# Sanoojan/REFace

Measured on AMD Instinct MI355X. Metric: 512x512 50-step DDIM images/sec, higher is better.
Workload: dtype bf16; 1 GPU; BASELINE configs[1]: 512x512, 50 DDIM steps, CFG scale 3.5, batch 8 per GPU, bf16 UNet + fp32 VAE decode (bf16x3 MFMA operands), seeded random-init REFace weights; id=c1:512x512:S50:B8:bf16, batch_per_gpu=8, global_batch=8, ddim_steps=50, latent=64, parallelism=dp1 (pairs sharded, no collective in the step loop)

## Files before the change

### reface_amd/csrc/common.h

```cpp
#pragma once
#include <hip/hip_runtime.h>
#include <stdint.h>
#include <stdio.h>
#include <stdlib.h>
#include <string.h>

#include "../../include/reface_hip.h"

typedef __attribute__((ext_vector_type(8))) __bf16 bf16x8_t;
typedef __attribute__((ext_vector_type(16))) float f32x16_t;
typedef __attribute__((ext_vector_type(4))) float f32x4_t;
typedef __attribute__((ext_vector_type(4))) uint32_t u32x4_t;
typedef __attribute__((ext_vector_type(2))) uint32_t u32x2_t;

typedef uint16_t bf16_t;
typedef _Float16 f16_t;
typedef __attribute__((ext_vector_type(8))) _Float16 f16x8_t;
typedef uint8_t fp8_t;

namespace rf {

void set_error(const char* fmt, ...);


// ... 117 lines not shown
template <> struct elem<f16_t> {
    static constexpr int VEC = 8;
    __device__ static __forceinline__ float load(const f16_t* p) { return (float)*p; }
    __device__ static __forceinline__ void store(f16_t* p, float v) { *p = (f16_t)v; }
};

template <typename T> __device__ __forceinline__ void unpack16(const u32x4_t& v, float* f);
template <> __device__ __forceinline__ void unpack16<float>(const u32x4_t& v, float* f) {
#pragma unroll
    for (int i = 0; i < 4; ++i) f[i] = as_f32( v[i]);
}
template <> __device__ __forceinline__ void unpack16<bf16_t>(const u32x4_t& v, float* f) {
#pragma unroll
    for (int i = 0; i < 4; ++i) {
        f[2 * i] = as_f32( v[i] << 16);
        f[2 * i + 1] = as_f32( v[i] & 0xffff0000u);
    }
}
template <> __device__ __forceinline__ void unpack16<f16_t>(const u32x4_t& v, float* f) {
#pragma unroll
    for (int i = 0; i < 4; ++i) {
        const uint32_t w = v[i];
        f[2 * i] = lo16<f16_t>(w);
        f[2 * i + 1] = hi16<f16_t>(w);
    }
}
template <typename T> __device__ __forceinline__ u32x4_t pack16(const float* f);
template <> __device__ __forceinline__ u32x4_t pack16<float>(const float* f) {
    u32x4_t v;
#pragma unroll
    for (int i = 0; i < 4; ++i) v[i] = as_u32( f[i]);
    return v;
}
template <> __device__ __forceinline__ u32x4_t pack16<bf16_t>(const float* f) {
    u32x4_t v;
#pragma unroll
    for (int i = 0; i < 4; ++i) v[i] = pack_bf2(f[2 * i], f[2 * i + 1]);
    return v;
}

template <> __device__ __forceinline__ u32x4_t pack16<f16_t>(const float* f) {
    u32x4_t v;
#pragma unroll
    for (int i = 0; i < 4; ++i) v[i] = pack_h2(f[2 * i], f[2 * i + 1]);
    return v;
}

template <typename T> __device__ __forceinline__ void mma16(f32x16_t& acc, const u32x4_t& a, const u32x4_t& b);
template <> __device__ __forceinline__ void mma16<bf16_t>(f32x16_t& acc, const u32x4_t& a, const u32x4_t& b) {
    acc = __builtin_amdgcn_mfma_f32_32x32x16_bf16(__builtin_bit_cast(bf16x8_t, a), __builtin_bit_cast(bf16x8_t, b), acc, 0, 0, 0);
}
template <> __device__ __forceinline__ void mma16<f16_t>(f32x16_t& acc, const u32x4_t& a, const u32x4_t& b) {
    acc = __builtin_amdgcn_mfma_f32_32x32x16_f16(__builtin_bit_cast(f16x8_t, a), __builtin_bit_cast(f16x8_t, b), acc, 0, 0, 0);
}

__device__ __forceinline__ float silu_exact(float x) {
    const float e = __builtin_amdgcn_exp2f(x * -1.4426950408889634f);
    return x * __builtin_amdgcn_rcpf(1.0f + e);
}
__device__ __forceinline__ float erf_rational(float x) {
    x = fminf(fmaxf(x, -4.0f), 4.0f);
    const float x2 = x * x;
    float a = -2.72614225801306e-10f;
    a = fmaf(a, x2, 2.77068142495902e-08f);
    a = fmaf(a, x2, -2.10102402082508e-06f);
    a = fmaf(a, x2, -5.69250639462346e-05f);
    a = fmaf(a, x2, -7.34990630326855e-04f);
    a = fmaf(a, x2, -2.95459980854025e-03f);
    a = fmaf(a, x2, -1.60960333262415e-02f);
    float b = -1.45660718464996e-05f;
    b = fmaf(b, x2, -2.13374055278905e-04f);
    b = fmaf(b, x2, -1.68282697438203e-03f);
    b = fmaf(b, x2, -7.37332916720468e-03f);
    b = fmaf(b, x2, -1.42647390514189e-02f);
    return x * a * __builtin_amdgcn_rcpf(b);
}
__device__ __forceinline__ float gelu_erf(float x) { return 0.5f * x * (1.0f + erf_rational(x * 0.70710678118654752440f)); }
__device__ __forceinline__ float gelu_sigmoid5(float x) {
    const float xc = __builtin_fminf(__builtin_fmaxf(x, -7.0f), 7.0f);
    const float x2 = xc * xc;
    const float u = xc * __builtin_fmaf(__builtin_fmaf(-0.0010142630f, x2, 0.10677572f), x2, 2.3011212f);
    return x * __builtin_amdgcn_rcpf(1.0f + __builtin_amdgcn_exp2f(-u));
}
template <typename T> __device__ __forceinline__ float gelu_for(float x) {
    if constexpr (sizeof(T) == 2) return gelu_sigmoid5(x);
    else return gelu_erf(x);
}
__device__ __forceinline__ float quick_gelu(float x) { return x / (1.0f + expf(-1.702f * x)); }

__device__ __forceinline__ void halfwave_reduce_scatter32(float (&gx)[32], int lrow) {
#pragma unroll
    for (int st = 0; st < 5; ++st) {
        const int m = 16 >> st, n = 16 >> st;
        const unsigned up = (lrow & m) ? 0xffffffffu : 0u;
#pragma unroll
        for (int k = 0; k < n; ++k) {
            const unsigned a = __float_as_uint(gx[k]), b = __float_as_uint(gx[k + n]);
            const float send = __uint_as_float((a & up) | (b & ~up));
            const float keep = __uint_as_float((b & up) | (a & ~up));
            gx[k] = keep + __shfl_xor(send, m, 64);
        }
    }
}

__device__ __forceinline__ float wave_sum(float v) {
    v += as_f32((uint32_t)__builtin_amdgcn_mov_dpp((int)as_u32(v), 0xB1, 0xF, 0xF, true));
// ... 36 lines not shown
```

### reface_amd/csrc/gemm.hip

```cpp
#include <cstdlib>
#include <type_traits>

#include "common.h"


namespace rf {
typedef float f32x2_t __attribute__((ext_vector_type(2)));

struct GemmParams {
    int M, N, K;
    const void* src0;
    const void* src1;
    int C0, Ctot, ld0, ld1;
    int Hin, Win, Hout, Wout, KH, KW, stride, pad_t, pad_l, ups;
    const void* W;
    int ldw;
    const float* bias;
    const float* rowvec;
    int rows_per_sample, ldv;
    const void* residual;
    int ldr, act;
    const float* act_vec;
    void* out;
    int ldo;
    float alpha;
    long long sA, sW, sO, sR;
    int tiles_m, tiles_n;
    unsigned a_bytes, w_bytes;
    int glds;
    int korder;
    int vec_ok;
    int splitk;
    float* ws;
    int pm, pn;
    int gn_rows;
    double* gn_part[2];
    int gn_cpg[2], gn_coff[2], gn_slot[2], gn_nch[2];
    int* plan;
    int epi2_ok;
    const float* wscale;
    void* oscale;
    int os_ld;
    const void* ascale;
    int as_ld;
    unsigned as_bytes;
    float* ln_out;
    int ln_out_parts;
    const float* ln_in;
    int ln_in_parts, ln_in_cols;
    float ln_eps;
    const float* ln_u;
    int x3;
    int lo_off;
    long long w_ps;
    const void* srcx;
    int ldx, xt0;
    unsigned x_bytes;
};

typedef __attribute__((ext_vector_type(2))) __bf16 bf16x2v_t;
__device__ __forceinline__ u32x4_t fp8x8_to_bf16x8(const u32x2_t& r, float scale) {
    u32x4_t o;
    o[0] = __builtin_bit_cast(uint32_t, __builtin_amdgcn_cvt_scalef32_pk_bf16_fp8(r[0], scale, false));
    o[1] = __builtin_bit_cast(uint32_t, __builtin_amdgcn_cvt_scalef32_pk_bf16_fp8(r[0], scale, true));
    o[2] = __builtin_bit_cast(uint32_t, __builtin_amdgcn_cvt_scalef32_pk_bf16_fp8(r[1], scale, false));
    o[3] = __builtin_bit_cast(uint32_t, __builtin_amdgcn_cvt_scalef32_pk_bf16_fp8(r[1], scale, true));
    return o;
}

template <typename T> struct MmaFrag;
template <> struct MmaFrag<bf16_t> {
    __device__ static __forceinline__ void mma(f32x16_t& acc, const u32x4_t& a, const u32x4_t& b) {
        acc = __builtin_amdgcn_mfma_f32_32x32x16_bf16(__builtin_bit_cast(bf16x8_t, a), __builtin_bit_cast(bf16x8_t, b), acc, 0, 0, 0);
    }
};
template <> struct MmaFrag<f16_t> {
    __device__ static __forceinline__ void mma(f32x16_t& acc, const u32x4_t& a, const u32x4_t& b) { mma16<f16_t>(acc, a, b); }
};
template <> struct MmaFrag<fp8_t> {
    __device__ static __forceinline__ void mma(f32x16_t&, const u32x4_t&, const u32x4_t&) {}
};
typedef int v8i_t __attribute__((ext_vector_type(8)));
__device__ __forceinline__ void mma_mx8(f32x16_t& acc, const u32x4_t& a0, const u32x4_t& a1, int sa, const u32x4_t& b0, const u32x4_t& b1, int sb) {
    const v8i_t a = {(int)a0[0], (int)a0[1], (int)a0[2], (int)a0[3], (int)a1[0], (int)a1[1], (int)a1[2], (int)a1[3]};
    const v8i_t b = {(int)b0[0], (int)b0[1], (int)b0[2], (int)b0[3], (int)b1[0], (int)b1[1], (int)b1[2], (int)b1[3]};
    asm volatile("s_nop 1\n\tv_mfma_scale_f32_32x32x64_f8f6f4 %0, %1, %2, %0, %3, %4 op_sel_hi:[0,0,0]" : "+v"(acc) : "v"(a), "v"(b), "v"(sa), "v"(sb));
}
template <> struct MmaFrag<float> {
    __device__ static __forceinline__ void mma(f32x16_t& acc, const u32x4_t& a, const u32x4_t& b) {
#pragma unroll
        for (int q = 0; q < 4; ++q)
            acc = __builtin_amdgcn_mfma_f32_32x32x2f32(as_f32( a[q]), as_f32( b[q]), acc, 0, 0, 0);
    }
};

__device__ __forceinline__ void lds_barrier() {
    asm volatile("s_waitcnt lgkmcnt(0)" ::: "memory");
    __builtin_amdgcn_s_barrier();
    asm volatile("" ::: "memory");
}

__device__ __forceinline__ int lds_off(int row, int slot) { return row * 128 + ((slot ^ ((row >> 1) & 7)) << 4); }

template <bool W8> __device__ __forceinline__ int w_stage(int t, int buf) { return W8 ? ((t >> 1) & 1) : buf; }
template <bool W8> __device__ __forceinline__ int w_soff(int t) { return (W8 ? (t >> 1) : t) * 128; }

template <typename TO> __device__ __forceinline__ void store_out(TO* p, float v);
template <> __device__ __forceinline__ void store_out<float>(float* p, float v) { *p = v; }
template <> __device__ __forceinline__ void store_out<bf16_t>(bf16_t* p, float v) { *p = f2bf(v); }
template <> __device__ __forceinline__ void store_out<f16_t>(f16_t* p, float v) { *p = (f16_t)v; }
template <typename TO> __device__ __forceinline__ float load_out(const TO* p);
template <> __device__ __forceinline__ float load_out<float>(const float* p) { return *p; }
template <> __device__ __forceinline__ float load_out<bf16_t>(const bf16_t* p) { return bf2f(*p); }
template <> __device__ __forceinline__ float load_out<f16_t>(const f16_t* p) { return (float)*p; }
template <typename X> struct is16 { static constexpr bool value = std::is_same<X, bf16_t>::value || std::is_same<X, f16_t>::value; };

template <typename T, typename TO, int WM, int WN, int TM, int TN, bool CONV, bool GLDS, int NST, int EPI = 0, bool W8 = false, int LNF = 0, bool HX = false>
__global__ __launch_bounds__(WM* WN * 64) void conv_gemm_kernel(const GemmParams p) {
    static_assert(LNF == 0 || (EPI == 1 && !CONV && !W8 && sizeof(T) == 2 && sizeof(TO) == 2), "LayerNorm folding: bf16 linear layers on the direct epilogue");
    static_assert(!HX || (CONV && GLDS && NST == 2 && sizeof(T) == 2 && !W8), "row-extended A tiles: bf16 3x3 convolutions on the two-stage direct-to-LDS loop");
    static_assert(EPI == 0 || GLDS, "the direct epilogue is built on the direct-to-LDS main loop");
    static_assert(!W8 || (GLDS && std::is_same<T, bf16_t>::value), "fp8 weights: bf16 activations on the direct-to-LDS main loop");
    constexpr bool A8 = std::is_same<T, fp8_t>::value;
    static_assert(!A8 || (GLDS && !W8 && NST == 2), "fp8 activations: direct-to-LDS main loop, two stages");
    constexpr int NT = WM * WN * 64;
    constexpr int BM = 32 * TM * WM;
    constexpr int BN = 32 * TN * WN;
    constexpr int VEC = elem<T>::VEC;
    constexpr int BK = 8 * VEC;
    constexpr int RPP = NT / 8;
    constexpr int AXR = HX ? ((BM * 5 / 4 + RPP - 1) / RPP) * RPP : BM;
    constexpr int AV = AXR / RPP;
    constexpr int BV = BN / RPP;
    static_assert(BM % RPP == 0 && BN % RPP == 0, "tile/threads mismatch");

    extern __shared__ __attribute__((aligned(16))) char smem[];
    char* const ldsA = smem;
    char* const ldsB = smem + NST * AXR * 128;
    char* const ldsS = smem + NST * (AXR + BN) * 128;

    const int tid = threadIdx.x;
    const int lane = tid & 63;
    const int wave = tid >> 6;
    const int wm = wave / WN, wn = wave % WN;

    int bid = blockIdx.x;
    {
        const int nwg = gridDim.x;
        const int q = nwg >> 3, r = nwg & 7, xcd = bid & 7, idx = bid >> 3;
        bid = (xcd < r ? xcd * (q + 1) : r * (q + 1) + (xcd - r) * q) + idx;
    }
    int tile_m, tile_n;
    {
        const int srow = p.pm * p.tiles_n;
        const int sr = bid / srow, rem = bid - sr * srow;
        const int h = min(p.pm, p.tiles_m - sr * p.pm);
        const int pw = h * p.pn;
        const int pc = rem / pw, r2 = rem - pc * pw;
        const int c = r2 / h;
        tile_m = sr * p.pm + (r2 - c * h);
        tile_n = pc * p.pn + c;
    }
    const int m0 = tile_m * BM, n0 = tile_n * BN;

    const long long zb = blockIdx.y;
    const T* src0 = (const T*)p.src0 + zb * p.sA;
    const T* src1 = (const T*)p.src1;
    const T* Wp = W8 ? (const T*)((const char*)p.W + zb * p.sW) : (const T*)p.W + zb * p.sW;
    if (!W8 && p.w_ps) Wp += (long long)(m0 / p.rows_per_sample) * p.w_ps;
    const int hw_in = p.Hin * p.Win;
    const int uph = (CONV && p.ups == 2) ? (m0 / hw_in) & 3 : 0;
// ... 368 lines not shown
                constexpr int cur = kk, nx = kk ^ 1, nkk = kk ^ 1;
                const char* const nA = kk == 0 ? curA : othA;
                const char* const nB = kk == 0 ? curB : othB;
                const char* const nS = kk == 0 ? curS : othS;
#pragma unroll
                for (int j = 0; j < JS8; ++j) mma_col(cur, j);
                if (kk == 1) {
                    asm volatile("s_waitcnt vmcnt(0) lgkmcnt(0)" ::: "memory");
                    __builtin_amdgcn_s_barrier();
                }
                ld_a(nx, nA, nS, nkk);
#pragma unroll
                for (int j = 0; j < JS8; ++j) ld_b(j, nB, nkk);
                __builtin_amdgcn_sched_barrier(0);
#pragma unroll
                for (int j = JS8; j < TN; ++j) {
                    mma_col(cur, j);
                    ld_b(j, nB, nkk);
                    if (kk == 1) {
                        constexpr int COLS = TN - JS8, PPC = (NP + COLS - 1) / COLS;
                        if (more) issue_pieces(stage, (j - JS8) * PPC, (j - JS8 + 1) * PPC < NP ? (j - JS8 + 1) * PPC : NP);
                    }
                    __builtin_amdgcn_sched_barrier(0);
                }
                __builtin_amdgcn_sched_barrier(0);
            };
            if (nk > 0) {
                issue_pieces(0, 0, AV);
                if (nk > 1) {
                    next_tile();
                    issue_pieces(1, 0, NP);
                    if (nk > 2) next_tile();
                    asm volatile("s_waitcnt vmcnt(%0)" ::"n"(NP + 1) : "memory");
                } else {
                    asm volatile("s_waitcnt vmcnt(0)" ::: "memory");
                }
                __builtin_amdgcn_s_barrier();
                ld_a(0, curA, curS, 0);
#pragma unroll
                for (int j = 0; j < TN; ++j) ld_b(j, curB, 0);
            }
            for (int kt = 0; kt < nk; ++kt) {
                const int stage = kt & 1;
                const bool more = kt + 2 < nk;
                phase8(integral_constant<int, 0>{}, stage, more);
                phase8(integral_constant<int, 1>{}, stage, more);
                if (kt + 3 < nk) next_tile();
                const char* t = curA; curA = othA; othA = t;
                t = curB; curB = othB; othB = t;
                t = curS; curS = othS; othS = t;
            }
            asm volatile("s_nop 15\n\ts_nop 15" ::: "memory");
            __syncthreads();
        } else {
        constexpr bool ROT = TM * TN > 8;
        constexpr int JS = ROT ? 2 : 0;
        u32x4_t fa[2][TM], fb[W8 ? 1 : 2][W8 ? 1 : TN];
        u32x2_t fbr[W8 ? 2 : 1][W8 ? TN : 1];
        float ws[W8 ? TN : 1];
        const int frag_sw = (lrow >> 1) & 7;
        const int brow = EPI == 1 ? (16 * ((lrow >> 2) & 1) + 4 * (lrow >> 3) + (lrow & 3)) : lrow;
        const int frag_swb = (brow >> 1) & 7;
        int fk[4], fkb[4];
#pragma unroll
        for (int kk = 0; kk < 4; ++kk) {
            fk[kk] = ((kk * 2 + lhalf) ^ frag_sw) << 4;
            fkb[kk] = W8 ? (((kk ^ frag_swb) << 4) + lhalf * 8) : (((kk * 2 + lhalf) ^ frag_swb) << 4);
        }
        if constexpr (W8) {
#pragma unroll
            for (int j = 0; j < TN; ++j) {
                const int n = n0 + (wn * TN + j) * 32 + brow;
                ws[j] = n < p.N ? p.wscale[n] : 1.0f;
            }
        }
        const char* curA = ldsA + (wm * TM) * 4096 + lrow * 128;
        int erow[TM];
        const char* hcb[TM];
        const char* hnb[TM];
        int hcs[TM], hns[TM], m_dx = 0, m_st = 0, m_len = 3, m_t = kb0_tiles;
        const int ks_[4] = {(0 + lhalf) << 4, (2 + lhalf) << 4, (4 + lhalf) << 4, (6 + lhalf) << 4};
        auto hx_set = [&](const char** hb, int* hs, int st, int dx) {
#pragma unroll
            for (int i = 0; i < TM; ++i) {
                const int e = erow[i] + dx;
                hb[i] = ldsA + st * (AXR * 128) + e * 128;
                hs[i] = ((e >> 1) & 7) << 4;
            }
        };
        if constexpr (HX) {
#pragma unroll
            for (int i = 0; i < TM; ++i) {
                const int pm = (wm * TM + i) * 32 + lrow, ir = pm / p.Wout;
                erow[i] = ir * (p.Wout + 2) + (pm - ir * p.Wout);
            }
            if (XT && kb0_tiles >= xt0) {
                m_len = 1;
                hx_set(hcb, hcs, 0, 1);
                hx_set(hnb, hns, 1, 1);
            } else {
                hx_set(hcb, hcs, 0, 0);
                hx_set(hnb, hns, 0, 1);
            }
        }
        const char* const wbase = ldsB + (wn * TN) * 4096 + brow * 128;
        const char* curB = wbase + w_stage<W8>(kb0_tiles, 0) * BN * 128;
// ... 927 lines not shown
            const double conc = 32.0, cap = 3.0 * 1024 * 1024;
            auto cost_of = [&](int h, int w) {
                const double nsr = (double)run / ((double)h * p.tiles_n) < 1.0 ? 1.0 : (double)run / ((double)h * p.tiles_n);
                const double npc = (double)p.tiles_n / w;
                const double a_t = (h * a_panel + w * w_panel <= cap) ? h * a_panel : npc * h * a_panel;
                return nsr * (a_t + p.tiles_n * w_panel);
            };
            double best = mfast ? cost_m : cost_n;
            const double strip_model = mfast ? cost_of(p.tiles_m, 1) : cost_of(1, p.tiles_n);
            if (strip_model > best) best = strip_model;
            for (int h = 2; h < p.tiles_m && h <= 32; h *= 2) {
                int w = (int)((conc + h - 1) / h);
                if (w < 1) w = 1;
                if (w >= p.tiles_n) continue;
                const double c = cost_of(h, w);
                if (c < 0.6 * best) { pm = h; pn = w; best = c / 0.6; }
            }
        }
        p.pm = pm;
        p.pn = pn;
    }
    constexpr bool FRAG_OK = (WM * WN == 8) || (TM * TN == 5) || (TM * TN >= 16) || std::is_same<T, fp8_t>::value;
    const bool frag = FRAG_OK && p.splitk > 1 && p.glds && p.epi2_ok && d->act == RF_ACT_NONE && !p.oscale && d->batch == 1 &&
                      (long long)p.splitk * p.tiles_m * p.tiles_n * BM * BN * 4 <= d->workspace_bytes;
    const int skr = sk_rows_for(p.M, p.N);
    const int st_rows = p.splitk > 1 ? (frag ? 32 : skr) : BM, st_cols = p.splitk > 1 ? (frag ? 32 * TN : SK_COLS) : BN;
    if (W8 || A8) RF_CHECK(p.glds, "rf_conv_gemm: fp8 operands need the direct-to-LDS main loop (one source, K and channel count multiples of the K tile)");
    if (p.oscale) {
        constexpr bool DOK = (WM * WN == 8) || (TM * TN == 5) || (TM * TN >= 16) || A8;
        RF_CHECK(DOK && TN % 2 == 0 && p.glds && p.epi2_ok && p.splitk == 1,
                 "rf_conv_gemm: fp8 output needs the direct epilogue (even TN, aligned rows, no split-K) -- this launch got a %d x %d tile", BM, BN);
    }
    constexpr bool DIRECT_OK = (WM * WN == 8) || (TM * TN == 5) || (TM * TN >= 16) || std::is_same<T, fp8_t>::value;
    const bool ep_common = p.glds && p.epi2_ok && p.splitk == 1 && (!p.rowvec || p.rows_per_sample % BM == 0) &&
                           (d->act == RF_ACT_NONE || d->act == RF_ACT_ADD_RELU || (d->act == RF_ACT_GEGLU && TN % 2 == 0));
    const bool direct = DIRECT_OK && ep_common && (p.gn_rows == 0 || d->act == RF_ACT_NONE);
    RF_CHECK(!hx || (HX_OK && conv && p.glds && p.KH == 3 && p.KW == 3 && p.stride == 1 && !p.ups && p.pad_t == 1 && p.pad_l == 1 && p.Hin == p.Hout &&
                     p.Win == p.Wout && p.Wout >= 16 && BM % p.Wout == 0 && (BM / p.Wout) * (p.Wout + 2) <= AXR_ &&
                     !(DEEP_OK && (long long)p.tiles_m * p.tiles_n * p.splitk <= 256)),
             "rf_conv_gemm: korder 2 (row-extended A tiles) needs a bf16 3x3 stride-1 pad-1 convolution, Wout >= 16, whose %d-row tile holds whole image rows (Wout = %d) "
             "and that does not take the 4-stage ring", BM, p.Wout);
    constexpr bool LN_OK = DIRECT_OK && sizeof(T) == 2 && sizeof(TO) == 2 && !W8 && !A8;
    RF_CHECK(!(p.ln_out || p.ln_in) || (LN_OK && !conv),
             "rf_conv_gemm: LayerNorm folding needs a bf16 linear layer on a direct-epilogue tile (this launch: %d x %d, conv %d)", BM, BN, (int)conv);
    RF_CHECK(!p.ln_in || !d->residual, "rf_conv_gemm: a LayerNorm consumer takes no residual");
    RF_CHECK(!p.ln_out || (direct && d->act == RF_ACT_NONE && p.N % (32 * TN) == 0 && p.ln_out_parts == p.N / (32 * TN)),
             "rf_conv_gemm: ln_stats_out needs the direct epilogue (no split-K, act NONE) and ln_out_parts = N / %d (got %d; direct %d)", 32 * TN, p.ln_out_parts, (int)direct);
    RF_CHECK(!p.ln_in || (direct && p.ln_u && p.ln_in_parts >= 1 && p.ln_in_cols >= 1 && p.ln_eps > 0.f && BN <= 320),
             "rf_conv_gemm: ln_stats_in needs the direct epilogue (no split-K), ln_u, ln_in_parts / ln_in_cols >= 1 and ln_eps > 0 (direct %d)", (int)direct);
    RF_CHECK(p.ups != 2 || (p.splitk == 1 && (p.Hin * p.Win) % BM == 0),
             "rf_conv_gemm: ups 2 needs Hin * Win = %d to be a multiple of the %d-row tile (a tile inside one phase of one sample) and no split-K (this launch: %d)",
             p.Hin * p.Win, BM, p.splitk);
    const bool deep = DEEP_OK && p.glds && !p.x3 && !hx && (long long)p.tiles_m * p.tiles_n * d->batch * p.splitk <= 256;
    if (p.plan) {
        p.plan[0] = st_rows; p.plan[1] = st_cols; p.plan[2] = p.splitk; p.plan[3] = BM; p.plan[4] = BN; p.plan[5] = 32 * TN;
        p.plan[6] = direct ? 1 : 0; p.plan[7] = frag ? 1 : 0;
        p.plan[8] = WM * WN; p.plan[9] = deep ? NSTD : 2; p.plan[10] = hx ? 1 : 0; p.plan[11] = p.glds ? 1 : 0; p.plan[12] = conv ? 1 : 0;
        p.plan[13] = p.ln_in ? 2 : (p.ln_out ? 1 : 0); p.plan[14] = p.pm; p.plan[15] = p.pn;
        p.plan[16] = p.splitk > 1 ? (frag ? 3 : (skr == 8 ? 1 : 2)) : 0;
        p.plan[17] = p.plan[18] = p.plan[19] = 0;
        p.plan[20] = p.tiles_m; p.plan[21] = p.tiles_n; p.plan[22] = p.plan[23] = 0;
        return 0;
    }
    if (p.gn_rows > 0) {
        RF_CHECK(p.gn_rows % st_rows == 0 && p.M % p.gn_rows == 0 && d->batch == 1 && d->act != RF_ACT_GEGLU,
                 "rf_conv_gemm: fused GroupNorm statistics need gn_rows %% %d == 0 (%d), batch 1, no GEGLU -- ask rf_conv_gemm_plan", st_rows, p.gn_rows);
        const int need = (p.gn_rows / st_rows) * ((p.N + st_cols - 1) / st_cols);
        for (int c = 0; c < 2; ++c)
            RF_CHECK(!p.gn_part[c] || (p.gn_cpg[c] > 0 && p.gn_slot[c] >= 0 && p.gn_slot[c] + need <= p.gn_nch[c]),
                     "rf_conv_gemm: GroupNorm consumer %d: cpg=%d slot=%d needs %d slots of %d", c, p.gn_cpg[c], p.gn_slot[c], need, p.gn_nch[c]);
    }
    dim3 grid(p.tiles_m * p.tiles_n, d->batch, p.splitk), block(WM * WN * 64);
    RF_CHECK(!p.oscale || direct, "rf_conv_gemm: fp8 output needs the direct epilogue (8-wave tile, aligned rows, no split-K)");
#define RF_LAUNCH_VARIANT_X(CONV_, GLDS_, EPI_, LNF_, HX_)                                                                      \
    {                                                                                                                            \
        constexpr int E_ = (EPI_ == 1 && DIRECT_OK) ? 1 : 0;                                                                     \
        if (GLDS_ && deep) {                                                                                                     \
            auto k = conv_gemm_kernel<T, TO, WM, WN, TM, TN, CONV_, GLDS_, (GLDS_ ? NSTD : 2), E_, (W8 && GLDS_), LNF_, false>; \
            RF_RAISE_LDS(k, smem_deep, "rf_conv_gemm");                                                                          \
            hipLaunchKernelGGL(k, grid, block, smem_deep, st, p);                                                                \
        } else {                                                                                                                 \
            auto k = conv_gemm_kernel<T, TO, WM, WN, TM, TN, CONV_, GLDS_, (GLDS_ ? NST : 2), E_, (W8 && GLDS_), LNF_, HX_>;    \
            constexpr int SM_ = HX_ ? smem_hx : smem;                                                                            \
            RF_RAISE_LDS(k, SM_, "rf_conv_gemm");                                                                                \
            hipLaunchKernelGGL(k, grid, block, SM_, st, p);                                                                      \
        }                                                                                                                        \
    }
#define RF_LAUNCH_VARIANT_LN(CONV_, GLDS_, EPI_, LNF_) RF_LAUNCH_VARIANT_X(CONV_, GLDS_, EPI_, LNF_, false)
#define RF_LAUNCH_VARIANT(CONV_, GLDS_, EPI_) RF_LAUNCH_VARIANT_LN(CONV_, GLDS_, EPI_, 0)
    const int esel = (direct || frag) ? 1 : 0;
    constexpr int smem_deep = NSTD * (BM + BN) * 128 > smem ? NSTD * (BM + BN) * 128 : smem;
    if constexpr (A8) {
        if (conv) { if (esel == 1) RF_LAUNCH_VARIANT(true, true, 1) else RF_LAUNCH_VARIANT(true, true, 0) }
        else { if (esel == 1) RF_LAUNCH_VARIANT(false, true, 1) else RF_LAUNCH_VARIANT(false, true, 0) }
    } else
    if (conv && p.glds) {
        if (hx) {
            if constexpr (HX_OK) {
                if (esel == 1) RF_LAUNCH_VARIANT_X(true, true, 1, 0, true)
                else RF_LAUNCH_VARIANT_X(true, true, 0, 0, true)
            }
        }
        else if (esel == 1) RF_LAUNCH_VARIANT(true, true, 1)
        else RF_LAUNCH_VARIANT(true, true, 0)
    } else if (conv) {
        RF_LAUNCH_VARIANT(true, false, 0)
    } else if (p.glds) {
        if (esel == 1) {
            if constexpr (LN_OK) {
                if (p.ln_in) RF_LAUNCH_VARIANT_LN(false, true, 1, 2)
                else if (p.ln_out) RF_LAUNCH_VARIANT_LN(false, true, 1, 1)
                else RF_LAUNCH_VARIANT(false, true, 1)
            } else RF_LAUNCH_VARIANT(false, true, 1)
        }
        else RF_LAUNCH_VARIANT(false, true, 0)
    } else {
        RF_LAUNCH_VARIANT(false, false, 0)
    }
#undef RF_LAUNCH_VARIANT
#undef RF_LAUNCH_VARIANT_LN
#undef RF_LAUNCH_VARIANT_X
    if (p.splitk > 1 && frag) {
        if constexpr (FRAG_OK)
            hipLaunchKernelGGL((splitk_reduce_frag_kernel<TO, WM, WN, TM, TN>), dim3(p.tiles_m * p.tiles_n, WM * WN * TM), dim3(64 * TN), 0, st, p);
    } else if (p.splitk > 1)
    {
        if (skr == 8) hipLaunchKernelGGL((splitk_reduce_kernel<TO, 8>), dim3((p.N + SK_COLS - 1) / SK_COLS, (p.M + 7) / 8), dim3(256), 0, st, p);
        else hipLaunchKernelGGL((splitk_reduce_kernel<TO, 32>), dim3((p.N + SK_COLS - 1) / SK_COLS, (p.M + 31) / 32), dim3(256), 0, st, p);
    }
    RF_LAUNCH_CHECK("rf_conv_gemm");
// ... 336 lines not shown
```

### reface_amd/csrc/norm.hip

```cpp
#include <stdarg.h>

#include "common.h"

namespace rf {

static thread_local char g_err[512] = "";
void set_error(const char* fmt, ...) {
    va_list ap;
    va_start(ap, fmt);
    vsnprintf(g_err, sizeof(g_err), fmt, ap);
    va_end(ap);
}

constexpr int GN_SLOTS = 4;
constexpr int GN_THREADS = 256;

template <typename T> struct gn_acc { typedef float type; };
template <> struct gn_acc<float> { typedef double type; };

template <typename T, int NS>
__global__ __launch_bounds__(GN_THREADS) void gn_stats_kernel(const T* __restrict__ x, int HW, int C, int ldx, int nchunks,
                                                              double* __restrict__ partial) {
    typedef typename gn_acc<T>::type acc_t;
    constexpr int VEC = elem<T>::VEC;
// ... 290 lines not shown
                if constexpr (sizeof(TO) == 1) {
                    quant_block8(y, orow + v * VEC, sc_out + (long long)(row0 + r) * lds_sc + (v >> 2), (v & 3) == 0);
                } else if constexpr (sizeof(TO) == sizeof(T)) {
                    *(u32x4_t*)(orow + v * VEC) = pack16<TO>(y);
                } else if constexpr (sizeof(TO) == 4) {
                    *(u32x4_t*)(orow + v * VEC) = pack16<float>(y);
                    *(u32x4_t*)(orow + v * VEC + 4) = pack16<float>(y + 4);
                } else {
                    u32x2_t h, l;
                    split4_bf16(y, h, l);
                    *(u32x2_t*)(orow + v * VEC) = h;
                    if (split) *(u32x2_t*)(orow + C + v * VEC) = l;
                }
            }
        }
    }
}

__global__ __launch_bounds__(256) void softmax_rows_kernel(float* __restrict__ x, int cols, int ld) {
    float* r = x + (long long)blockIdx.x * ld;
    __shared__ float red[4];
    float m = -INFINITY;
    for (int c = threadIdx.x * 4; c < cols; c += 1024) {
        const f32x4_t v = *(const f32x4_t*)(r + c);
        m = fmaxf(fmaxf(fmaxf(m, v[0]), fmaxf(v[1], v[2])), v[3]);
    }
    m = wave_max(m);
    if ((threadIdx.x & 63) == 0) red[threadIdx.x >> 6] = m;
    __syncthreads();
    m = fmaxf(fmaxf(red[0], red[1]), fmaxf(red[2], red[3]));
    __syncthreads();
    float s = 0.f;
    for (int c = threadIdx.x * 4; c < cols; c += 1024) {
        const f32x4_t v = *(const f32x4_t*)(r + c);
        s += expf(v[0] - m) + expf(v[1] - m) + expf(v[2] - m) + expf(v[3] - m);
    }
    s = wave_sum(s);
    if ((threadIdx.x & 63) == 0) red[threadIdx.x >> 6] = s;
    __syncthreads();
    const float inv = 1.0f / (red[0] + red[1] + red[2] + red[3]);
    for (int c = threadIdx.x * 4; c < cols; c += 1024) {
        f32x4_t v = *(const f32x4_t*)(r + c);
#pragma unroll
        for (int e = 0; e < 4; ++e) v[e] = expf(v[e] - m) * inv;
        *(f32x4_t*)(r + c) = v;
    }
}

}

using namespace rf;

extern "C" const char* rf_last_error(void) { return rf::g_err; }
extern "C" int rf_version(void) { return 111; }

static int gn_check(const char* name, int dtype, int C, int ldx, int nchunks) {
    const int vec = dtype == RF_F32 ? 4 : 8;
    RF_CHECK(dtype == RF_F32 || dtype == RF_BF16 || dtype == RF_F16, "%s: bad dtype %d", name, dtype);
    RF_CHECK(C % 32 == 0 && C % vec == 0 && ldx % vec == 0, "%s: C=%d ld=%d must be multiples of 32 and %d", name, C, ldx, vec);
    RF_CHECK(C / vec <= GN_SLOTS * GN_THREADS, "%s: C=%d too large", name, C);
    RF_CHECK(nchunks >= 1, "%s: nchunks=%d", name, nchunks);
    return 0;
}

extern "C" int rf_groupnorm_stats(int dtype, const void* x, int B, int HW, int C, int ldx, int nchunks, double* partial, void* stream) {
    if (gn_check("rf_groupnorm_stats", dtype, C, ldx, nchunks)) return 1;
    RF_CHECK(x && partial && B > 0 && HW > 0, "rf_groupnorm_stats: bad arguments");
    dim3 grid(nchunks, B);
    const int vec = dtype == RF_F32 ? 4 : 8;
    const int nvec = C / vec, TV = nvec < GN_THREADS ? nvec : GN_THREADS, PL = GN_THREADS / TV;
    const size_t smem = (size_t)2 * PL * C * sizeof(double);
    RF_CHECK(smem <= 64 * 1024, "rf_groupnorm_stats: C=%d needs %zu B of LDS", C, smem);
    const int ns = (nvec + GN_THREADS - 1) / GN_THREADS;
#define GN_STATS_(T, NS_) hipLaunchKernelGGL((gn_stats_kernel<T, NS_>), grid, dim3(GN_THREADS), smem, (hipStream_t)stream, (const T*)x, HW, C, ldx, nchunks, partial)
#define GN_STATS(T) { if (ns <= 1) GN_STATS_(T, 1); else if (ns <= 2) GN_STATS_(T, 2); else GN_STATS_(T, GN_SLOTS); }
    if (dtype == RF_F32) GN_STATS(float)
    else if (dtype == RF_F16) GN_STATS(f16_t)
    else GN_STATS(bf16_t)
#undef GN_STATS
#undef GN_STATS_
    RF_LAUNCH_CHECK("rf_groupnorm_stats");
    return 0;
}

__global__ __launch_bounds__(GN_THREADS) void gn_finalize_kernel(const double* __restrict__ in, int nchunks, double* __restrict__ out) {
    const int b = blockIdx.x, g = threadIdx.x & 31, part = threadIdx.x >> 5;
    __shared__ double red[GN_THREADS][2];
    double a = 0.0, q = 0.0;
    for (int c = part; c < nchunks; c += GN_THREADS / 32) {
        const double* pp = in + (((long long)b * nchunks + c) * 32 + g) * 2;
        a += pp[0];
        q += pp[1];
    }
    red[threadIdx.x][0] = a;
    red[threadIdx.x][1] = q;
    __syncthreads();
    if (threadIdx.x < 32) {
        double sa = 0.0, sq = 0.0;
        for (int k = 0; k < GN_THREADS / 32; ++k) { sa += red[threadIdx.x + 32 * k][0]; sq += red[threadIdx.x + 32 * k][1]; }
        out[((long long)b * 32 + threadIdx.x) * 2] = sa;
        out[((long long)b * 32 + threadIdx.x) * 2 + 1] = sq;
    }
}

extern "C" int rf_groupnorm_finalize(const double* partial_in, int B, int nchunks, double* partial_out, void* stream) {
    RF_CHECK(partial_in && partial_out && B > 0 && nchunks >= 1, "rf_groupnorm_finalize: bad arguments");
    hipLaunchKernelGGL(gn_finalize_kernel, dim3(B), dim3(GN_THREADS), 0, (hipStream_t)stream, partial_in, nchunks, partial_out);
// ... 241 lines not shown
```

### reface_amd/ops.py

```python
import ctypes as C
import threading

import torch

from . import _lib
from ._lib import (ACT_ADD_RELU, ACT_GEGLU, ACT_GELU, ACT_NONE, ACT_PRELU, ACT_QUICK_GELU, ACT_RELU, ACT_SIGMOID, ACT_SILU, RF_BF16, RF_BF16X3, RF_F16, RF_F32,
                   RF_FP8_E4M3, AttnInDesc, ConvGemmDesc, FfnDesc, StemDesc)

LOG2E = 1.4426950408889634
LN2 = 0.6931471805599453


def code(dt):
    if dt == torch.float32:
        return RF_F32
    if dt == torch.bfloat16:
        return RF_BF16
    if dt == torch.float16:
        return RF_F16
    raise TypeError(f"unsupported dtype {dt}")


H16 = (torch.bfloat16, torch.float16)

# ... 498 lines not shown

def gn_chunks(B, HW):
    n = max(1, min(GN_MAX_CHUNKS, HW // 32))
    while B * n > 512 and n > 1:
        n //= 2
    return n


def _gn_out_code(x, out, split):
    if split:
        assert x.dtype == torch.float32 and out.dtype == torch.bfloat16 and out.shape[-1] == 2 * x.shape[-1]
        return RF_BF16X3
    return code(out.dtype)


def groupnorm_stats(x, partial, name="groupnorm"):
    lib = _lib.load()
    B, H, W_, Cc = x.shape
    n = gn_chunks(B, H * W_)
    _require_gpu(x, partial)
    assert partial.dtype == torch.float64 and partial.numel() >= B * n * 64
    return Launch(lib.rf_groupnorm_stats, (code(x.dtype), _p(x), B, H * W_, Cc, x.stride(2), n, _p(partial)), (x, partial), name + ".stats"), n


def groupnorm(x, gamma, beta, out, partial, *, eps, silu, split=False, name="groupnorm"):
    lib = _lib.load()
    B, H, W_, Cc = x.shape
    HW = H * W_
    n = gn_chunks(B, HW)
    assert partial.dtype == torch.float64 and partial.numel() >= B * n * 64
    a = Launch(lib.rf_groupnorm_stats, (code(x.dtype), _p(x), B, HW, Cc, x.stride(2), n, _p(partial)), (x, partial), name + ".stats")
    if isinstance(out, Fp8Act):
        return [a, groupnorm_apply(x, gamma, beta, out, partial, n, eps=eps, silu=silu, name=name)]
    _require_gpu(x, gamma, beta, out, partial)
    b = Launch(lib.rf_groupnorm_apply, (code(x.dtype), _p(x), B, HW, Cc, x.stride(2), n, _p(partial), _p(gamma), _p(beta),
                                        float(eps), int(bool(silu)), _gn_out_code(x, out, split), _p(out), out.stride(2)),
               (x, partial, gamma, beta, out), name + ".apply")
    return [a, b]


def gemm_plan(launch):
    lib = _lib.load()
    bm, bn, sk = C.c_int32(0), C.c_int32(0), C.c_int32(0)
    _lib.check(lib.rf_conv_gemm_plan(C.byref(launch.keep[0]), C.byref(bm), C.byref(bn), C.byref(sk)), launch.name + ".plan")
    return bm.value, bn.value, sk.value


def gemm_plan2(launch):
    lib = _lib.load()
    info = (C.c_int32 * 8)()
    _lib.check(lib.rf_conv_gemm_plan2(C.byref(launch.keep[0]), info), launch.name + ".plan2")
    pl = dict(zip(("stat_rows", "stat_cols", "splitk", "bm", "bn", "wave_cols", "direct", "frag"), (int(v) for v in info)))
    pl["gemm_kernels"] = 2 if pl["frag"] & 2 else 1
    pl["frag"] &= 1
    return pl


REDUCE_KINDS = ("none", "stripe8", "stripe32", "frag")


def gemm_plan3(launch):
    lib = _lib.load()
    info = (C.c_int32 * 24)()
    _lib.check(lib.rf_conv_gemm_plan3(C.byref(launch.keep[0]), info), launch.name + ".plan3")
    v = [int(x) for x in info]
    pl = dict(zip(("stat_rows", "stat_cols", "splitk", "bm", "bn", "wave_cols", "direct", "frag"), v[:8]))
    pl["gemm_kernels"] = 2 if pl["frag"] & 2 else 1
    pl["frag"] &= 1
    pl.update(waves=v[8], stages=v[9], hx=v[10], glds=v[11], conv=v[12], ln_role=v[13], pm=v[14], pn=v[15], reduce=REDUCE_KINDS[v[16]],
              tiles_m=v[20], tiles_n=v[21], tail=((v[17], v[18], v[19], v[23]) if pl["gemm_kernels"] == 2 else None), split_n=v[22])
    return pl


def fold_layernorm_linear(w, gamma, beta, bias, dtype):
    wf = w.float()
    w2 = (wf * gamma.float()[None, :]).to(dtype).contiguous()
    u = w2.float().sum(dim=1).contiguous()
    b2 = wf @ beta.float()
    if bias is not None:
        b2 = b2 + bias.float()
    return w2, u, b2.contiguous()


def layernorm_fold(producers, consumer, *, eps, C_):
    cd = consumer.keep[0]
    M = cd.M
    plans = []
    for l, row0, rows in producers:
        d = l.keep[0]
        if l.fn.__name__ != "rf_conv_gemm" or d.N != C_ or d.act != ACT_NONE or d.M != rows:
            return None
        pl = gemm_plan2(l)
        if not pl["direct"] or pl["splitk"] != 1 or C_ % pl["wave_cols"]:
            return None
        plans.append(pl["wave_cols"])
    if len(set(plans)) != 1 or sum(r for _, _, r in producers) != M:
        return None
    wc = plans[0]
    parts = C_ // wc
    stats = torch.zeros((M, parts, 2), dtype=torch.float32, device=consumer.keep[1].device)
    try:
        for l, row0, rows in producers:
            d = l.keep[0]
            d.ln_stats_out, d.ln_out_parts = stats[row0:].data_ptr(), parts
            gemm_plan2(l)
        cd.ln_stats_in, cd.ln_in_parts, cd.ln_in_cols, cd.ln_eps = stats.data_ptr(), parts, wc, float(eps)
        gemm_plan2(consumer)
    except _lib.RefaceHipError:
        for l, _, _ in producers:
            l.keep[0].ln_stats_out, l.keep[0].ln_out_parts = None, 0
        cd.ln_stats_in, cd.ln_in_parts, cd.ln_in_cols, cd.ln_eps = None, 0, 0, 0.0
        return None
    for l, _, _ in producers:
        l.keep = tuple(l.keep) + (stats,)
    consumer.keep = tuple(consumer.keep) + (stats,)
    return stats


def fuse_groupnorm_stats(x, producers):
    B, H, W_, Cc = x.shape
# ... 658 lines not shown
```

Baseline: 10.27 images/s.

## Add 16x16x32 MFMA main loop for deep-K bf16/fp16 conv GEMMs

New measurement: 10.30 images/s, median of 6. No clear change (+0.3%).

```diff
diff --git a/reface_amd/csrc/common.h b/reface_amd/csrc/common.h
--- a/reface_amd/csrc/common.h
+++ b/reface_amd/csrc/common.h
@@ -193,6 +193,13 @@
 }
 template <> __device__ __forceinline__ void mma16<f16_t>(f32x16_t& acc, const u32x4_t& a, const u32x4_t& b) {
     acc = __builtin_amdgcn_mfma_f32_32x32x16_f16(__builtin_bit_cast(f16x8_t, a), __builtin_bit_cast(f16x8_t, b), acc, 0, 0, 0);
+}
+template <typename T> __device__ __forceinline__ void mma16x16(f32x4_t& acc, const u32x4_t& a, const u32x4_t& b);
+template <> __device__ __forceinline__ void mma16x16<bf16_t>(f32x4_t& acc, const u32x4_t& a, const u32x4_t& b) {
+    acc = __builtin_amdgcn_mfma_f32_16x16x32_bf16(__builtin_bit_cast(bf16x8_t, a), __builtin_bit_cast(bf16x8_t, b), acc, 0, 0, 0);
+}
+template <> __device__ __forceinline__ void mma16x16<f16_t>(f32x4_t& acc, const u32x4_t& a, const u32x4_t& b) {
+    acc = __builtin_amdgcn_mfma_f32_16x16x32_f16(__builtin_bit_cast(f16x8_t, a), __builtin_bit_cast(f16x8_t, b), acc, 0, 0, 0);
 }
 
 __device__ __forceinline__ float silu_exact(float x) {
diff --git a/reface_amd/csrc/gemm.hip b/reface_amd/csrc/gemm.hip
--- a/reface_amd/csrc/gemm.hip
+++ b/reface_amd/csrc/gemm.hip
@@ -68,6 +68,13 @@
     return o;
 }
 
+template <int I, int N, typename F> __device__ __forceinline__ void static_for(F&& f) {
+    if constexpr (I < N) {
+        f(std::integral_constant<int, I>{});
+        static_for<I + 1, N>(f);
+    }
+}
+
 template <typename T> struct MmaFrag;
 template <> struct MmaFrag<bf16_t> {
     __device__ static __forceinline__ void mma(f32x16_t& acc, const u32x4_t& a, const u32x4_t& b) {
@@ -115,8 +122,9 @@
 template <> __device__ __forceinline__ float load_out<f16_t>(const f16_t* p) { return (float)*p; }
 template <typename X> struct is16 { static constexpr bool value = std::is_same<X, bf16_t>::value || std::is_same<X, f16_t>::value; };
 
-template <typename T, typename TO, int WM, int WN, int TM, int TN, bool CONV, bool GLDS, int NST, int EPI = 0, bool W8 = false, int LNF = 0, bool HX = false>
+template <typename T, typename TO, int WM, int WN, int TM, int TN, bool CONV, bool GLDS, int NST, int EPI = 0, bool W8 = false, int LNF = 0, bool HX = false, bool M16 = false>
 __global__ __launch_bounds__(WM* WN * 64) void conv_gemm_kernel(const GemmParams p) {
+    static_assert(!M16 || (GLDS && is16<T>::value && std::is_same<T, TO>::value && !W8 && LNF == 0), "16x16x32 main loop: bf16 / fp16 in and out on the direct-to-LDS loop");
     static_assert(LNF == 0 || (EPI == 1 && !CONV && !W8 && sizeof(T) == 2 && sizeof(TO) == 2), "LayerNorm folding: bf16 linear layers on the direct epilogue");
     static_assert(!HX || (CONV && GLDS && NST == 2 && sizeof(T) == 2 && !W8), "row-extended A tiles: bf16 3x3 convolutions on the two-stage direct-to-LDS loop");
     static_assert(EPI == 0 || GLDS, "the direct epilogue is built on the direct-to-LDS main loop");
@@ -591,6 +599,158 @@
             }
             asm volatile("s_nop 15\n\ts_nop 15" ::: "memory");
             __syncthreads();
+        } else if constexpr (M16) {
+        using std::integral_constant;
+        constexpr int RB = 2 * TM, CB = 2 * TN, NG = 2 * CB;
+        constexpr int RING = TM > 1 ? 4 : CB;
+        constexpr int TB = NG - RING;
+        constexpr int TA = CB - 4;
+        static_assert(NG % RING == 0 && RING >= 4 && RING <= CB && TA >= 0, "W fragment ring");
+        auto mma_blk = [&](f32x16_t& blk, int q, const u32x4_t& a, const u32x4_t& b) {
+            f32x4_t c = {blk[4 * q], blk[4 * q + 1], blk[4 * q + 2], blk[4 * q + 3]};
+            mma16x16<T>(c, a, b);
+#pragma unroll
+            for (int e = 0; e < 4; ++e) blk[4 * q + e] = c[e];
+        };
+        u32x4_t fa[2][RB], fb[RING];
+        const int p16 = lane & 15, kg = lane >> 4;
+        const int ppi = 8 * ((p16 >> 2) & 1) + 4 * (p16 >> 3) + (p16 & 3);
+        const int arow = EPI == 1 ? p16 : ppi;
+        const int wrow = EPI == 1 ? 16 * (p16 >> 3) + 4 * ((p16 >> 2) & 1) + (p16 & 3) : p16;
+        constexpr int WHALF = EPI == 1 ? 1024 : 2048;
+        const int ksl[2] = {(kg >> 1) + 6 * (kg & 1), 2 + (kg >> 1) + 2 * (kg & 1)};
+        int fkA[2], fkW[2][2];
+#pragma unroll
+        for (int ks = 0; ks < 2; ++ks) {
+            fkA[ks] = (ksl[ks] ^ ((arow >> 1) & 7)) << 4;
+            fkW[ks][0] = (ksl[ks] ^ ((wrow >> 1) & 7)) << 4;
+            fkW[ks][1] = EPI == 1 ? fkW[ks][0] ^ 64 : fkW[ks][0];
+        }
+        const char* curA = ldsA + (wm * TM) * 4096 + arow * 128;
+        const char* othA = curA + BM * 128;
+        const char* const wbase = ldsB + (wn * TN) * 4096 + wrow * 128;
+        const char* curB = wbase;
+        const char* othB = wbase + BN * 128;
+        int hb[RB];
+        int f_col = 0, f_dx = 0, f_st = 0, f_len = 3, f_t = kb0_tiles;
+        if constexpr (HX) {
+            if (XT && kb0_tiles >= xt0) { f_len = 1; f_col = 1; }
+#pragma unroll
+            for (int ab = 0; ab < RB; ++ab) {
+                const int pm = (wm * TM) * 32 + ab * 16 + arow, ir = pm / p.Wout;
+                hb[ab] = (ir * (p.Wout + 2) + (pm - ir * p.Wout) + f_col) * 128;
+            }
+        }
+        auto hx_next = [&]() {
+            const int st0 = f_st, col0 = f_col;
+            ++f_t;
+            if (++f_dx == f_len) { f_dx = 0; f_st ^= 1; if (XT && f_t >= xt0) f_len = 1; }
+            f_col = (XT && f_t >= xt0) ? 1 : f_dx;
+            const int d = __builtin_amdgcn_readfirstlane((f_st - st0) * (AXR * 128) + (f_col - col0) * 128);
+#pragma unroll
+            for (int ab = 0; ab < RB; ++ab) hb[ab] += d;
+        };
+        auto load_a = [&](int set, int ks, const char* base) {
+#pragma unroll
+            for (int ab = 0; ab < RB; ++ab) {
+                if constexpr (HX) fa[set][ab] = *(const u32x4_t*)(ldsA + hb[ab] + ((ksl[ks] ^ ((hb[ab] >> 8) & 7)) << 4));
+                else fa[set][ab] = *(const u32x4_t*)(base + (ab >> 1) * 4096 + (ab & 1) * 2048 + fkA[ks]);
+            }
+        };
+        auto load_w = [&](auto G, const char* base) {
+            constexpr int g = decltype(G)::value, ks = g / CB, cb = g % CB;
+            fb[g % RING] = *(const u32x4_t*)(base + (cb >> 1) * 4096 + (cb & 1) * WHALF + fkW[ks][cb & 1]);
+        };
+        auto group = [&](auto TT, int stage, bool more, bool deep) {
+            constexpr int t = decltype(TT)::value, ks = t / CB, cb = t % CB;
+            const u32x4_t bj = fb[t % RING];
+#pragma unroll
+            for (int ab = 0; ab < RB; ++ab) {
+                if constexpr (EPI == 1) mma_blk(acc[ab >> 1][cb >> 1], 2 * (cb & 1) + (ab & 1), bj, fa[ks][ab]);
+                else mma_blk(acc[ab >> 1][cb >> 1], 2 * (ab & 1) + (cb & 1), fa[ks][ab], bj);
+            }
+            if constexpr (t == TA) load_a(1, 1, curA);
+            if constexpr (t + RING < NG) {
+                load_w(integral_constant<int, t + RING>{}, curB);
+            } else if constexpr (t == TB + 1) {
+                if (NST > 2 && deep) asm volatile("s_waitcnt vmcnt(%0) lgkmcnt(0)" ::"n"((NST - 2) * NP) : "memory");
+                else asm volatile("s_waitcnt vmcnt(0) lgkmcnt(0)" ::: "memory");
+                __builtin_amdgcn_s_barrier();
+                load_a(0, 0, othA);
+                load_w(integral_constant<int, 0>{}, othB);
+                load_w(integral_constant<int, 1>{}, othB);
+            } else if constexpr (t > TB + 1) {
+                load_w(integral_constant<int, t + RING - NG>{}, othB);
+            }
+            if constexpr (t > TB) {
+                constexpr int COLS = RING - 1, PPC = (NP + COLS - 1) / COLS, c = t - TB - 1;
+                if (more) issue_pieces(stage, c * PPC, (c + 1) * PPC < NP ? (c + 1) * PPC : NP);
+            }
+            if constexpr (HX) {
+                if constexpr (t == TA + 1) hx_next();
+            }
+            __builtin_amdgcn_sched_barrier(0);
+        };
+        if (nk > 0) {
+            issue_pieces(0, 0, AV);
+            if constexpr (NST > 2) {
+#pragma unroll
+                for (int s = 1; s < NST; ++s)
+                    if (s < nk) {
+                        next_tile();
+                        issue_pieces(s, 0, NP);
+                    }
+                if (nk > NST) next_tile();
+                if (nk >= NST) asm volatile("s_waitcnt vmcnt(%0)" ::"n"((NST - 1) * NP) : "memory");
+                else asm volatile("s_waitcnt vmcnt(0)" ::: "memory");
+            } else if (nk > 1) {
+                next_tile();
+                issue_pieces(1, 0, NP);
+                if (nk > 2) next_tile();
+                asm volatile("s_waitcnt vmcnt(%0)" ::"n"(HX ? BV : NP) : "memory");
+            } else {
+                asm volatile("s_waitcnt vmcnt(0)" ::: "memory");
+            }
+            __builtin_amdgcn_s_barrier();
+            load_a(0, 0, curA);
+            static_for<0, RING>([&](auto G) { load_w(G, curB); });
+        }
+        if constexpr (NST > 2) {
+            const char* const baseA = curA;
+            int sc = 0, so = 1;
+            for (int kt = 0; kt < nk; ++kt) {
+                const bool more = kt + NST < nk, deep = kt + NST - 1 < nk;
+                static_for<0, NG>([&](auto TT) { group(TT, sc, more, deep); });
+                if (kt + NST + 1 < nk) next_tile();
+                sc = so;
+                so = so + 1 == NST ? 0 : so + 1;
+                curA = othA; othA = baseA + so * (BM * 128);
+                curB = othB; othB = wbase + so * (BN * 128);
+            }
+        } else {
+            for (int kt = 0; kt < nk; ++kt) {
+                const int stage = kt & 1;
+                const bool more = kt + 2 < nk;
+                static_for<0, NG>([&](auto TT) { group(TT, stage, more, false); });
+                if (kt + 3 < nk) next_tile();
+                const char* t = curA; curA = othA; othA = t;
+                t = curB; curB = othB; othB = t;
+            }
+        }
+#pragma unroll
+        for (int i = 0; i < TM; ++i)
+#pragma unroll
+            for (int j = 0; j < TN; ++j)
+#pragma unroll
+                for (int rb = 0; rb < 2; ++rb)
+#pragma unroll
+                    for (int r = 0; r < 4; ++r) {
+                        const auto sw = __builtin_amdgcn_permlane16_swap(as_u32(acc[i][j][8 * rb + r]), as_u32(acc[i][j][8 * rb + 4 + r]), false, false);
+                        acc[i][j][8 * rb + r] = as_f32(sw[0]);
+                        acc[i][j][8 * rb + 4 + r] = as_f32(sw[1]);
+                    }
+        __builtin_amdgcn_sched_barrier(0);
+        __syncthreads();
         } else {
         constexpr bool ROT = TM * TN > 8;
         constexpr int JS = ROT ? 2 : 0;
@@ -1624,9 +1784,19 @@
              "rf_conv_gemm: ups 2 needs Hin * Win = %d to be a multiple of the %d-row tile (a tile inside one phase of one sample) and no split-K (this launch: %d)",
              p.Hin * p.Win, BM, p.splitk);
     const bool deep = DEEP_OK && p.glds && !p.x3 && !hx && (long long)p.tiles_m * p.tiles_n * d->batch * p.splitk <= 256;
+    constexpr bool M16_OK = is16<T>::value && std::is_same<T, TO>::value && !W8 && WM == 4 && TN >= 4 && TM * TN != 10;
+    constexpr bool M16_E1 = M16_OK;
+    constexpr int M16_MIN_K = 2560;
+    bool m16 = false;
+    if (M16_OK && p.glds && !p.x3 && !p.ln_in && !p.ln_out) {
+        const int bk_ = 128 / (int)sizeof(T), nk_ = p.K / bk_;
+        int per = (nk_ + p.splitk - 1) / p.splitk;
+        if (p.splitk > 1 && hx) per = (per + 2) / 3 * 3;
+        m16 = per * bk_ >= M16_MIN_K && (!(direct || frag) || M16_E1);
+    }
     if (p.plan) {
         p.plan[0] = st_rows; p.plan[1] = st_cols; p.plan[2] = p.splitk; p.plan[3] = BM; p.plan[4] = BN; p.plan[5] = 32 * TN;
-        p.plan[6] = direct ? 1 : 0; p.plan[7] = frag ? 1 : 0;
+        p.plan[6] = direct ? 1 : 0; p.plan[7] = (frag ? 1 : 0) | (m16 ? 4 : 0);
         p.plan[8] = WM * WN; p.plan[9] = deep ? NSTD : 2; p.plan[10] = hx ? 1 : 0; p.plan[11] = p.glds ? 1 : 0; p.plan[12] = conv ? 1 : 0;
         p.plan[13] = p.ln_in ? 2 : (p.ln_out ? 1 : 0); p.plan[14] = p.pm; p.plan[15] = p.pn;
         p.plan[16] = p.splitk > 1 ? (frag ? 3 : (skr == 8 ? 1 : 2)) : 0;
@@ -1647,7 +1817,27 @@
 #define RF_LAUNCH_VARIANT_X(CONV_, GLDS_, EPI_, LNF_, HX_)                                                                      \
     {                                                                                                                            \
         constexpr int E_ = (EPI_ == 1 && DIRECT_OK) ? 1 : 0;                                                                     \
-        if (GLDS_ && deep) {                                                                                                     \
+        constexpr bool M_ = M16_OK && GLDS_ && LNF_ == 0 && (E_ == 0 || M16_E1);                                                 \
+        bool done_ = false;                                                                                                      \
+        if constexpr (M_ && DEEP_OK) {                                                                                           \
+            if (m16 && deep) {                                                                                                   \
+                auto k = conv_gemm_kernel<T, TO, WM, WN, TM, TN, CONV_, GLDS_, (GLDS_ ? NSTD : 2), E_, false, 0, false, true>;   \
+                RF_RAISE_LDS(k, smem_deep, "rf_conv_gemm");                                                                      \
+                hipLaunchKernelGGL(k, grid, block, smem_deep, st, p);                                                            \
+                done_ = true;                                                                                                    \
+            }                                                                                                                    \
+        }                                                                                                                        \
+        if constexpr (M_) {                                                                                                      \
+            if (m16 && !done_) {                                                                                                    \
+                auto k = conv_gemm_kernel<T, TO, WM, WN, TM, TN, CONV_, GLDS_, (GLDS_ ? NST : 2), E_, false, 0, HX_, true>;      \
+                constexpr int SM_ = HX_ ? smem_hx : smem;                                                                        \
+                RF_RAISE_LDS(k, SM_, "rf_conv_gemm");                                                                            \
+                hipLaunchKernelGGL(k, grid, block, SM_, st, p);                                                                  \
+                done_ = true;                                                                                                    \
+            }                                                                                                                    \
+        }                                                                                                                        \
+        if (done_) {                                                                                                             \
+        } else if (GLDS_ && deep) {                                                                                                     \
             auto k = conv_gemm_kernel<T, TO, WM, WN, TM, TN, CONV_, GLDS_, (GLDS_ ? NSTD : 2), E_, (W8 && GLDS_), LNF_, false>; \
             RF_RAISE_LDS(k, smem_deep, "rf_conv_gemm");                                                                          \
             hipLaunchKernelGGL(k, grid, block, smem_deep, st, p);                                                                \
diff --git a/reface_amd/csrc/norm.hip b/reface_amd/csrc/norm.hip
--- a/reface_amd/csrc/norm.hip
+++ b/reface_amd/csrc/norm.hip
@@ -366,7 +366,7 @@
 using namespace rf;
 
 extern "C" const char* rf_last_error(void) { return rf::g_err; }
-extern "C" int rf_version(void) { return 111; }
+extern "C" int rf_version(void) { return 112; }
 
 static int gn_check(const char* name, int dtype, int C, int ldx, int nchunks) {
     const int vec = dtype == RF_F32 ? 4 : 8;
diff --git a/reface_amd/ops.py b/reface_amd/ops.py
--- a/reface_amd/ops.py
+++ b/reface_amd/ops.py
@@ -574,6 +574,7 @@
     _lib.check(lib.rf_conv_gemm_plan2(C.byref(launch.keep[0]), info), launch.name + ".plan2")
     pl = dict(zip(("stat_rows", "stat_cols", "splitk", "bm", "bn", "wave_cols", "direct", "frag"), (int(v) for v in info)))
     pl["gemm_kernels"] = 2 if pl["frag"] & 2 else 1
+    pl["mfma16"] = 1 if pl["frag"] & 4 else 0
     pl["frag"] &= 1
     return pl
 
@@ -588,6 +589,7 @@
     v = [int(x) for x in info]
     pl = dict(zip(("stat_rows", "stat_cols", "splitk", "bm", "bn", "wave_cols", "direct", "frag"), v[:8]))
     pl["gemm_kernels"] = 2 if pl["frag"] & 2 else 1
+    pl["mfma16"] = 1 if pl["frag"] & 4 else 0
     pl["frag"] &= 1
     pl.update(waves=v[8], stages=v[9], hx=v[10], glds=v[11], conv=v[12], ln_role=v[13], pm=v[14], pn=v[15], reduce=REDUCE_KINDS[v[16]],
               tiles_m=v[20], tiles_n=v[21], tail=((v[17], v[18], v[19], v[23]) if pl["gemm_kernels"] == 2 else None), split_n=v[22])
```
